# martellab-sri/ModalTune

Hardware: AMD Instinct MI355X
Metric: slides/sec (train step) at 10k patches x 1536-d (higher is better)
Workload: dtype f16; 1 GPU; Prov-GigaPath ModalAdapter train step, 10000 patches x 1536-d, 6 pathways -> 64 gene tokens + 1 task token, 3 task passes, fp16 operands / fp32 accumulate, 1 slide per GPU per step, task passes as two concurrent groups (B = 2 | 1 on two HIP streams), train mode: Dropout(0.25) on the embedded input and both backbone branches, DropPath(0..0.1) per layer and on the Extractor FFN (Philox masks regener; patches=10000, parallelism=dp1, dropout=True

## Files before the change

modaltune_amd/csrc/attn_combine.hip:

```cpp
#include "attn_common.h"

namespace {

__global__ __launch_bounds__(192) void dilated_attn_bwd_combine_kernel(const h16* __restrict__ ws, Plan p, h16* __restrict__ dqkv) {
  const long M = (long)p.B * p.N;
  const int t = threadIdx.x;
  const int col = t * 12, which = col / DM, h = (col % DM) / HD, d0 = col % HD;
  for (long m = blockIdx.x; m < M; m += gridDim.x) {
    const int pos = (int)(m % p.N);
    float acc[12];
#pragma unroll
    for (int e = 0; e < 12; ++e) acc[e] = 0.f;
#pragma unroll
    for (int br = 0; br < MT_MAX_BRANCHES; ++br) {
      if (br < p.nbranch) {
        const int dr = p.ratio[br], sg = p.seg[br], hb = H / dr;
        const int j = pos / sg, loc = pos - j * sg;
        if (loc % dr == h / hb) {
          const h16* src = ws + p.ws_off[br] + ((m * 3 + which) * hb + (h % hb)) * HD + d0;
          const h16x4 a0 = *reinterpret_cast<const h16x4*>(src), a1 = *reinterpret_cast<const h16x4*>(src + 4),
                      a2 = *reinterpret_cast<const h16x4*>(src + 8);
#pragma unroll
          for (int e = 0; e < 4; ++e) { acc[e] += (float)a0[e]; acc[4 + e] += (float)a1[e]; acc[8 + e] += (float)a2[e]; }
        }
      }
    }
    h16* dst = dqkv + m * QKV_LD + col;
#pragma unroll
    for (int k = 0; k < 3; ++k) {
      const h16x4 o = {(h16)acc[4 * k], (h16)acc[4 * k + 1], (h16)acc[4 * k + 2], (h16)acc[4 * k + 3]};
      *reinterpret_cast<h16x4*>(dst + 4 * k) = o;
    }
  }
}

constexpr int CMB_PIECES = QKV_LD / 8;
constexpr int CMB_GRID_MAX = 2048;
template <int NB>
__global__ __launch_bounds__(256) void dilated_attn_bwd_combine_inplace_kernel(const h16* __restrict__ ws, Plan p, int db, h16* dqkv) {
  const long M = (long)p.B * p.N;
  const int lane = threadIdx.x & 63, wave = __builtin_amdgcn_readfirstlane(threadIdx.x >> 6);
  const LivePasses lp = live_passes(p);
  const long m_end = min(M, (long)lp.b1 * p.N);
  for (long m = (long)lp.b0 * p.N + (long)blockIdx.x * 4 + wave; m < m_end; m += (long)gridDim.x * 4) {
    const int pos = (int)((unsigned)m % (unsigned)p.N);
    h16* row = dqkv + m * QKV_LD;
    int lo[NB], hbs[NB], str[NB];
    const h16* src[NB];
#pragma unroll
    for (int br = 0; br < NB; ++br) {
      const bool sparse = br < p.nbranch && br != db;
      const int dr = sparse ? p.ratio[br] : 1, sg = sparse ? p.seg[br] : 1, hb = H / dr;
      const int loc = pos % sg;
      lo[br] = (loc % dr) * hb;
      hbs[br] = sparse ? hb : 0;
      str[br] = hb * HD;
      src[br] = br == db ? row : ws + (sparse ? p.ws_off[br] + (m * 3 * hb - lo[br]) * HD : 0);
    }
#pragma unroll 1
    for (int it = 0; it < (CMB_PIECES + 63) / 64; ++it) {
      const int piece = it * 64 + lane;
      const int which = piece / (DM / 8), hp = piece - which * (DM / 8), h = hp / 6;
      bool cov[NB], any = false;
#pragma unroll
      for (int br = 0; br < NB; ++br) {
        cov[br] = piece < CMB_PIECES && (unsigned)(h - lo[br]) < (unsigned)hbs[br];
        any |= cov[br];
      }
      h16x8 v[NB];
#pragma unroll
      for (int br = 0; br < NB; ++br) {
        if (br == db) cov[br] = any;
        const h16* a = cov[br] ? src[br] + (which * str[br] + hp * 8) : ws;
        v[br] = *reinterpret_cast<const h16x8*>(a);
      }
      float acc[8];
#pragma unroll
      for (int e = 0; e < 8; ++e) acc[e] = 0.f;
#pragma unroll
      for (int br = 0; br < NB; ++br) {
        const h16x8 x = sel8(cov[br], v[br]);
#pragma unroll
        for (int e = 0; e < 8; ++e) acc[e] += (float)x[e];
      }
      if (any) {
        h16x8 o;
#pragma unroll
        for (int e = 0; e < 8; ++e) o[e] = (h16)acc[e];
        *reinterpret_cast<h16x8*>(row + piece * 8) = o;
      }
    }
  }
}

}

void mt_attn::launch_bwd_combine(const void* ws, const MtDilatedPlan* plan, mt_half* dqkv, hipStream_t s) {
  const Plan p = make_plan(plan, 128);
  const long M = (long)p.B * p.N;
  hipLaunchKernelGGL(dilated_attn_bwd_combine_kernel, dim3((int)min(M, 16384L)), dim3(192), 0, s, (const h16*)ws, p, (h16*)dqkv);
}

void mt_attn::launch_bwd_combine_inplace(const void* ws, const MtDilatedPlan* plan, mt_half* dqkv, const int* live, hipStream_t s) {
  const Plan p = make_plan(plan, 128, live);
  const long M = (long)p.B * p.N;
  const int db = dense_branch_host(plan);
  const dim3 grid((int)min((M + 3) / 4, (long)CMB_GRID_MAX));
  if (p.nbranch <= 5)
    hipLaunchKernelGGL(dilated_attn_bwd_combine_inplace_kernel<5>, grid, dim3(256), 0, s, (const h16*)ws, p, db, (h16*)dqkv);
  else
    hipLaunchKernelGGL(dilated_attn_bwd_combine_inplace_kernel<MT_MAX_BRANCHES>, grid, dim3(256), 0, s, (const h16*)ws, p, db, (h16*)dqkv);
}
```

Before: 25.83 slides/s.

## Stage sparse-branch dQKV rows into LDS with contiguous lane loads in combine

Adds a combine kernel that loads each row's sparse-branch workspace gradients as one contiguous run into per-wave LDS via global_load_lds, so every lane issues a coalesced 16-byte load instead of scattered masked loads. The dense-branch row is prefetched into registers while those loads are in flight, then the kernel gathers from LDS and sums in fp32. The aim is to cut uncoalesced global traffic and load latency in this memory-bound backward combine. In exchange it relies on hand-placed waitcnt and inline-asm barriers, uses 17 KB of LDS per block, and only applies when the staged pieces fit within 272.

After: 25.88 slides/s, median of 5. No clear change (+0.2%).

```diff
diff --git a/modaltune_amd/csrc/attn_combine.hip b/modaltune_amd/csrc/attn_combine.hip
--- a/modaltune_amd/csrc/attn_combine.hip
+++ b/modaltune_amd/csrc/attn_combine.hip
@@ -93,6 +93,120 @@
   }
 }
 
+constexpr int CMB_STAGE_PIECES = 272;
+constexpr int CMB_STAGE_LOADS = (CMB_STAGE_PIECES + 63) / 64;
+constexpr int CMB_ITERS = (CMB_PIECES + 63) / 64;
+constexpr int CMB_NB = 5;
+MT_DEVINL int opaque(int v) { asm volatile("" : "+v"(v)); return v; }
+struct CombineStage { int start[CMB_NB + 1]; long off_bytes[CMB_NB]; };
+__global__ __launch_bounds__(256) void dilated_attn_bwd_combine_dense_lanes_kernel(const h16* __restrict__ ws, Plan p, int db, CombineStage cs, h16* dqkv) {
+  constexpr int NB = CMB_NB;
+  __shared__ __attribute__((aligned(16))) h16 stage[4][CMB_STAGE_PIECES * 8];
+  const long M = (long)p.B * p.N;
+  const int lane = threadIdx.x & 63, wave = __builtin_amdgcn_readfirstlane(threadIdx.x >> 6);
+  h16* const st = stage[wave];
+  int start[NB + 1];
+  long off0[NB];
+#pragma unroll
+  for (int br = 0; br <= NB; ++br) start[br] = __builtin_amdgcn_readfirstlane(cs.start[br]);
+#pragma unroll
+  for (int br = 0; br < NB; ++br)
+    off0[br] = ((long)__builtin_amdgcn_readfirstlane((int)(cs.off_bytes[br] >> 32)) << 32) | (unsigned)__builtin_amdgcn_readfirstlane((int)cs.off_bytes[br]);
+  int row_bytes[CMB_STAGE_LOADS];
+  long off_bytes[CMB_STAGE_LOADS];
+#pragma unroll
+  for (int i = 0; i < CMB_STAGE_LOADS; ++i) {
+    const int c = i * 64 + lane;
+    row_bytes[i] = 0; off_bytes[i] = 0;
+#pragma unroll
+    for (int br = 0; br < NB; ++br) {
+      const bool in = c >= start[br] && c < start[br + 1];
+      row_bytes[i] = in ? (start[br + 1] - start[br]) * 16 : row_bytes[i];
+      off_bytes[i] = in ? off0[br] + (long)(c - start[br]) * 16 : off_bytes[i];
+    }
+  }
+  const LivePasses lp = live_passes(p);
+  const long m_end = min(M, (long)lp.b1 * p.N);
+  for (long m = (long)lp.b0 * p.N + (long)blockIdx.x * 4 + wave; m < m_end; m += (long)gridDim.x * 4) {
+    const int pos = (int)((unsigned)m % (unsigned)p.N);
+    h16* row = dqkv + m * QKV_LD;
+    int lo[NB], hbs[NB], sbase[NB];
+#pragma unroll
+    for (int br = 0; br < NB; ++br) {
+      const bool sparse = br < p.nbranch && br != db;
+      const int dr = sparse ? p.ratio[br] : 1, sg = sparse ? p.seg[br] : 1, hb = H / dr;
+      const int loc = pos % sg;
+      lo[br] = (loc % dr) * hb;
+      hbs[br] = sparse ? hb : 0;
+      sbase[br] = start[br] - lo[br] * 6;
+    }
+    asm volatile("s_waitcnt lgkmcnt(0)" ::: "memory");
+#pragma unroll
+    for (int i = 0; i < CMB_STAGE_LOADS; ++i)
+      if (row_bytes[i] != 0) {
+        const char* a = reinterpret_cast<const char*>(ws) + off_bytes[i] + (unsigned long)(unsigned)m * (unsigned)row_bytes[i];
+        __builtin_amdgcn_global_load_lds((const __attribute__((address_space(1))) void*)a,
+                                         (__attribute__((address_space(3))) void*)(st + i * 512), 16, 0, 0);
+      }
+    h16x8 dv[CMB_ITERS];
+#pragma unroll
+    for (int it = 0; it < CMB_ITERS; ++it) {
+      const int piece = it * 64 + opaque(lane);
+      const int which = piece / (DM / 8), h = (piece - which * (DM / 8)) / 6;
+      bool any = false;
+#pragma unroll
+      for (int br = 0; br < NB; ++br) any |= piece < CMB_PIECES && (unsigned)(h - lo[br]) < (unsigned)hbs[br];
+      dv[it] = *reinterpret_cast<const h16x8*>(any ? row + piece * 8 : ws);
+    }
+    __builtin_amdgcn_s_waitcnt(0x0F70);
+    asm volatile("" ::: "memory");
+#pragma unroll
+    for (int it = 0; it < CMB_ITERS; ++it) {
+      const int piece = it * 64 + opaque(lane);
+      const int which = piece / (DM / 8), hp = piece - which * (DM / 8), h = hp / 6;
+      bool cov[NB], any = false;
+      h16x8 v[NB];
+#pragma unroll
+      for (int br = 0; br < NB; ++br) {
+        cov[br] = piece < CMB_PIECES && (unsigned)(h - lo[br]) < (unsigned)hbs[br];
+        any |= cov[br];
+        v[br] = *reinterpret_cast<const h16x8*>(st + (cov[br] ? sbase[br] + which * 6 * hbs[br] + hp : 0) * 8);
+      }
+#pragma unroll
+      for (int br = 0; br < NB; ++br) {
+        cov[br] = br == db ? any : cov[br];
+        v[br] = br == db ? dv[it] : v[br];
+      }
+      float acc[8];
+#pragma unroll
+      for (int e = 0; e < 8; ++e) acc[e] = 0.f;
+#pragma unroll
+      for (int br = 0; br < NB; ++br) {
+        const h16x8 x = sel8(cov[br], v[br]);
+#pragma unroll
+        for (int e = 0; e < 8; ++e) acc[e] += (float)x[e];
+      }
+      if (any) {
+        h16x8 o;
+#pragma unroll
+        for (int e = 0; e < 8; ++e) o[e] = (h16)acc[e];
+        *reinterpret_cast<h16x8*>(row + piece * 8) = o;
+      }
+      asm volatile("" ::: "memory");
+    }
+  }
+}
+
+CombineStage make_combine_stage(const Plan& p, int db) {
+  CombineStage cs;
+  cs.start[0] = 0;
+  for (int b = 0; b < CMB_NB; ++b) {
+    cs.start[b + 1] = cs.start[b] + (b < p.nbranch && b != db ? 18 * (H / p.ratio[b]) : 0);
+    cs.off_bytes[b] = b < p.nbranch ? p.ws_off[b] * 2 : 0;
+  }
+  return cs;
+}
+
 }
 
 void mt_attn::launch_bwd_combine(const void* ws, const MtDilatedPlan* plan, mt_half* dqkv, hipStream_t s) {
@@ -106,7 +220,10 @@
   const long M = (long)p.B * p.N;
   const int db = dense_branch_host(plan);
   const dim3 grid((int)min((M + 3) / 4, (long)CMB_GRID_MAX));
-  if (p.nbranch <= 5)
+  const CombineStage cs = make_combine_stage(p, db);
+  if (p.nbranch <= CMB_NB && cs.start[CMB_NB] <= CMB_STAGE_PIECES)
+    hipLaunchKernelGGL(dilated_attn_bwd_combine_dense_lanes_kernel, grid, dim3(256), 0, s, (const h16*)ws, p, db, cs, (h16*)dqkv);
+  else if (p.nbranch <= 5)
     hipLaunchKernelGGL(dilated_attn_bwd_combine_inplace_kernel<5>, grid, dim3(256), 0, s, (const h16*)ws, p, db, (h16*)dqkv);
   else
     hipLaunchKernelGGL(dilated_attn_bwd_combine_inplace_kernel<MT_MAX_BRANCHES>, grid, dim3(256), 0, s, (const h16*)ws, p, db, (h16*)dqkv);
```
